# minjiyoon/MMGL

Hardware: AMD Instinct MI355X
Metric: train samples/sec (OPT-1.3B flamingo, 16 neighbors) (higher is better)
Workload: dtype bf16; 1 GPU; opt-1.3b context=all neighbor_mode=embedding peft=flamingo, 11+5 neighbors x 4 tokens, T=512+128, roberta-base + clip-vit-base-patch16 frozen encoders, full train step (fwd+bwd+exchange+AdamW); per_gpu_batch=64, global_batch=64, seq_len=640, neighbor_keys=64, trainable_params=216736520, parallelism=dp1

## Files before the change

include/mmgl_hip.h:

```cpp
#ifndef MMGL_HIP_H
#define MMGL_HIP_H

#include <stddef.h>
#include <stdint.h>

#ifdef __cplusplus
extern "C" {
#endif

enum { MMGL_F32 = 0, MMGL_BF16 = 1 };
enum { MMGL_OK = 0, MMGL_ERR_INVALID = 1, MMGL_ERR_UNSUPPORTED = 2, MMGL_ERR_HIP = 3 };
enum { MMGL_ACT_NONE = 0, MMGL_ACT_RELU = 1 };

const char* mmgl_last_error(void);
int mmgl_version(void);

int mmgl_xattn_fwd(const void* q, const void* k, const void* v, const uint8_t* key_valid,
                   void* out, float* lse, int B, int H, int T, int S, int D, int dtype, void* stream);

size_t mmgl_xattn_bwd_workspace(int B, int H, int T, int S, int D);
int mmgl_xattn_bwd(const void* dout, const void* q, const void* k, const void* v, const float* lse,
                   const uint8_t* key_valid, void* dq, void* dk, void* dv,
                   void* workspace, size_t workspace_bytes,
                   int B, int H, int T, int S, int D, int dtype, void* stream);
// ... 51 lines not shown
size_t mmgl_norm_bwd_workspace(int rows, int cols);
int mmgl_layernorm_bwd(const void* dy, const void* x, const void* gamma, const float* mean, const float* rstd,
                       void* dx, float* dgamma, float* dbeta, void* workspace, size_t workspace_bytes,
                       int rows, int cols, int dtype, void* stream);

int mmgl_rmsnorm_fwd(const void* x, const void* gamma, void* y, float* rstd,
                     int rows, int cols, float eps, int dtype, void* stream);
int mmgl_rmsnorm_bwd(const void* dy, const void* x, const void* gamma, const float* rstd,
                     void* dx, float* dgamma, void* workspace, size_t workspace_bytes,
                     int rows, int cols, int dtype, void* stream);

int mmgl_add_rmsnorm_fwd(const void* x, const void* res, const void* gamma, void* sum_out, void* y, float* rstd,
                         int rows, int cols, float eps, int dtype, void* stream);
int mmgl_add_rmsnorm_bwd(const void* dy, const void* dsum, const void* sum, const void* gamma, const float* rstd,
                         void* dres, float* dgamma, void* workspace, size_t workspace_bytes,
                         int rows, int cols, int dtype, void* stream);

int mmgl_gated_residual_fwd(const void* residual, const void* x, const float* gate, void* y,
                            size_t n, float p_drop, uint64_t seed, int dtype, void* stream);
size_t mmgl_gated_residual_bwd_workspace(size_t n);
int mmgl_gated_residual_bwd(const void* dy, const void* x, const float* gate, void* dx, float* dgate,
                            void* workspace, size_t workspace_bytes,
                            size_t n, float p_drop, uint64_t seed, int dtype, void* stream);

int mmgl_linear_fwd(const void* x, const void* W, const void* bias, void* y,
                    int M, int N, int K, int act, float out_scale, int dtype, void* stream);
size_t mmgl_linear_bwd_workspace(int M, int N, int K, int act, int dtype);
int mmgl_linear_bwd(const void* dy, const void* y, const void* x, const void* W, void* dx, void* dW, void* dbias,
                    void* workspace, size_t workspace_bytes, int M, int N, int K, int act, float out_scale,
                    int accumulate, int mask_dx, int dtype, void* stream);

int mmgl_lora_linear_fwd(const void* x, const void* W, const void* bias, const void* A, const void* Bm,
                         void* y, void* xa, int M, int N, int K, int r, float scale, int dtype, void* stream);
size_t mmgl_lora_linear_bwd_workspace(int M, int N, int K, int r, int dtype);
int mmgl_lora_linear_bwd(const void* dy, const void* x, const void* xa, const void* W, const void* A,
                         const void* Bm, void* dx, void* dA, void* dB, void* dyb, void* workspace,
                         size_t workspace_bytes, int M, int N, int K, int r, float scale, int accumulate,
                         int dtype, void* stream);

int mmgl_neighbor_interleave_fwd(const void* text_emb, const void* vis_emb, const int64_t* text_loc,
                                 const int64_t* img_loc, const int64_t* text_pos, const int64_t* img_pos,
                                 void* out_emb, uint8_t* out_valid, int B, int Nt, int Ni, int n_tok, int d,
                                 int dtype, void* stream);
int mmgl_neighbor_interleave_bwd(const void* d_out_emb, const int64_t* text_loc, const int64_t* img_loc,
                                 void* d_text_emb, void* d_vis_emb, int B, int Nt, int Ni, int n_tok, int d,
                                 int dtype, void* stream);

int mmgl_cross_entropy_fwd(const void* logits, const int64_t* labels, float* row_lse, float* row_loss,
                           float* loss_sum, float* count, int rows, int V, int64_t ignore_index, int dtype,
                           void* stream);
int mmgl_cross_entropy_bwd(const void* logits, const int64_t* labels, const float* row_lse,
                           const float* count, const float* dloss, void* dlogits,
                           int rows, int V, int64_t ignore_index, int dtype, void* stream);

int mmgl_position_ids(const int64_t* attention_mask, int64_t* pos, int B, int T, void* stream);

int mmgl_adamw_step(void* param, float* master, const void* grad, float* exp_avg, float* exp_avg_sq, size_t n,
                    float lr, float beta1, float beta2, float eps, float weight_decay, int step,
                    float grad_scale, int dtype, void* stream);

int mmgl_gemm_nt_fast(int M, int N, int K, int ldx, int ldw, int ldy, int dtype);
size_t mmgl_gemm_nt_workspace(int M, int N, int K, int ldx, int ldw, int ldy, int dtype);
int mmgl_gemm_nt(const void* x, int ldx, const void* W, int ldw, const void* bias, const void* residual, const void* zmask,
                 void* y, int ldy, int M, int N, int K, int act, float out_scale, void* workspace, size_t workspace_bytes,
                 int dtype, void* stream);
int mmgl_relu_bwd(const void* dy, const void* y, void* out, size_t n, int dtype, void* stream);
int mmgl_gemm_nt_rowk(const void* x, int ldx, const void* W, int ldw, void* y, int ldy, int M, int N, int K, int K_short,
                      int m_full, int dtype, void* stream);
int mmgl_gemm_nt_rowk_item(int G, int n_long, int n_short, int q, int wg, int it);
int mmgl_gemm_set_tile_counter(void* counter);
void* mmgl_gemm_get_tile_counter(void);
size_t mmgl_gemm_nt_relu_bits_bytes(int M, int N, int K, int ldx, int ldw, int ldy, int dtype);
int mmgl_gemm_nt_relu_bits(const void* x, int ldx, const void* W, int ldw, const void* bias, void* y, int ldy, void* bits_out,
                           int M, int N, int K, float out_scale, int dtype, void* stream);
int mmgl_gemm_nt_masked(const void* x, int ldx, const void* W, int ldw, const void* bits_in, void* y, int ldy, int M, int N, int K,
                        float out_scale, int dtype, void* stream);

int mmgl_rope_inplace(void* buf, const float* cos_sin, size_t rows, int T, int H, int D, int ld, int nblk, int backward,
                      int dtype, void* stream);
int mmgl_rope(const void* src, void* dst, const float* cos_sin, size_t rows, int T, int H, int D, int ld, int nblk, int nall,
              int backward, int dtype, void* stream);
int mmgl_swiglu_fwd(const void* gate_up, void* y, size_t M, int F, int dtype, void* stream);
int mmgl_swiglu_bwd(const void* dy, const void* gate_up, void* dgate_up, size_t M, int F, int dtype, void* stream);

int mmgl_encattn_fwd(const void* q, const void* k, const void* v, const int32_t* cu_seqlens, void* out, int nseq,
                     int H, int D, int ld_in, int ld_out, int max_len, int q_rows, int dtype, void* stream);
int mmgl_add_layernorm_fwd(const void* x, const void* res, const void* gamma, const void* beta, void* sum_out,
                           void* y, float* mean, float* rstd, int rows, int cols, float eps, float p_drop, uint64_t seed,
                           int dtype, void* stream);
int mmgl_add_layernorm_bwd(const void* dy, const void* dsum, const void* sum, const void* gamma, const float* mean,
                           const float* rstd, void* dres, void* dx, float* dgamma, float* dbeta, void* workspace,
                           size_t workspace_bytes, int rows, int cols, float p_drop, uint64_t seed, int dtype,
                           void* stream);
int mmgl_layernorm_tiles_fwd(const void* x, const void* gamma, const void* beta, void* y, void* yc, const int32_t* rowmap,
                             float* mean, float* rstd, int rows, int cols, int crows, float eps, int dtype, void* stream);
int mmgl_add_layernorm_tiles_fwd(const void* x, const void* res, const void* gamma, const void* beta, void* sum_out, void* y,
                                 void* yc, const int32_t* rowmap, float* mean, float* rstd, int rows, int cols, int crows,
                                 float eps, float p_drop, uint64_t seed, int dtype, void* stream);
int mmgl_add_layernorm_rows_bwd(const void* dy, const int32_t* dy_rows, const void* dsum, const void* sum, const void* gamma,
                                const float* mean, const float* rstd, void* dres, void* dx, float* dgamma, float* dbeta,
                                void* workspace, size_t workspace_bytes, int rows, int cols, float p_drop, uint64_t seed,
                                int dtype, void* stream);
int mmgl_activation_fwd(const void* x, void* y, size_t n, int act, int dtype, void* stream);
int mmgl_scale(const void* x, const float* scale, void* y, size_t n, int dtype, void* stream);

enum { MMGL_COMM_I64 = 2 };
// ... 87 lines not shown
```

mmgl_amd/_lib.py:

```python
import ctypes
import os

import torch

_HERE = os.path.dirname(os.path.abspath(__file__))
LIB_PATH = os.environ.get("MMGL_LIB_PATH") or os.path.join(_HERE, "libmmgl_hip.so")

ABI_VERSION = 110
F32, BF16 = 0, 1
ACT_NONE, ACT_RELU = 0, 1
_ERR_INVALID, _ERR_UNSUPPORTED, _ERR_HIP = 1, 2, 3

c_void_p, c_int, c_float, c_size_t, c_u64, c_i64 = (ctypes.c_void_p, ctypes.c_int, ctypes.c_float, ctypes.c_size_t,
                                                    ctypes.c_uint64, ctypes.c_int64)
P, I, F, Z, U, L = c_void_p, c_int, c_float, c_size_t, c_u64, c_i64

SIGNATURES = {
    "mmgl_last_error": (ctypes.c_char_p, []),
    "mmgl_version": (I, []),
    "mmgl_xattn_fwd": (I, [P, P, P, P, P, P, I, I, I, I, I, I, P]),
    "mmgl_xattn_bwd_workspace": (Z, [I, I, I, I, I]),
    "mmgl_xattn_bwd": (I, [P, P, P, P, P, P, P, P, P, P, Z, I, I, I, I, I, I, P]),
    "mmgl_selfattn_fwd": (I, [P, P, P, P, P, P, I, I, I, I, I, I, P]),
    "mmgl_selfattn_bwd_workspace": (Z, [I, I, I]),
    "mmgl_selfattn_bwd": (I, [P, P, P, P, P, P, P, P, P, P, P, Z, I, I, I, I, I, I, I, P]),
    "mmgl_selfattn_prefix_fwd": (I, [P, P, P, P, P, P, I, I, I, I, I, I, I, I, P]),
    "mmgl_selfattn_prefix_bwd": (I, [P, P, P, P, P, P, P, P, P, P, P, Z, I, I, I, I, I, I, I, I, I, I, P]),
    "mmgl_selfattn_tiles_fwd": (I, [P, P, P, P, P, P, P, I, I, I, I, I, I, I, I, P]),
    "mmgl_selfattn_tiles_bwd": (I, [P, P, P, P, P, P, P, P, P, P, P, P, Z, I, I, I, I, I, I, I, I, I, I, P]),
    "mmgl_selfattn_tiles_rows_bwd": (I, [P, P, P, P, P, P, P, P, P, P, P, P, P, Z, I, I, I, I, I, I, I, I, I, I, I, P]),
    "mmgl_selfattn_gqa_fwd": (I, [P, P, P, P, P, P, I, I, I, I, I, I, I, I, P]),
    "mmgl_selfattn_gqa_bwd_workspace": (Z, [I, I, I, I, I, I]),
    "mmgl_selfattn_gqa_bwd": (I, [P, P, P, P, P, P, P, P, P, P, P, Z, I, I, I, I, I, I, I, I, I, I, P]),
    "mmgl_attn_general_fwd": (I, [P, P, P, P, P, P, P, P, I, I, I, I, I, I, F, U, I, P]),
    "mmgl_attn_general_bwd_workspace": (Z, [I, I, I]),
    "mmgl_attn_general_bwd": (I, [P, P, P, P, P, P, P, P, P, P, P, Z, I, I, I, I, I, I, F, U, I, P]),
    "mmgl_attn_dropout_mask": (I, [P, I, I, I, I, F, U, P]),
    "mmgl_attn_relbias_fwd": (I, [P, P, P, P, P, P, P, P, I, I, I, I, I, I, I, I, I, F, U, I, P]),
    "mmgl_attn_relbias_bwd_workspace": (Z, [I, I, I, I]),
    "mmgl_attn_relbias_bwd": (I, [P, P, P, P, P, P, P, P, P, P, P, P, P, P, Z, I, I, I, I, I, I, I, I, I, F, U, I, P]),
    "mmgl_layernorm_fwd": (I, [P, P, P, P, P, P, I, I, F, I, P]),
    "mmgl_norm_bwd_workspace": (Z, [I, I]),
    "mmgl_layernorm_bwd": (I, [P, P, P, P, P, P, P, P, P, Z, I, I, I, P]),
    "mmgl_rmsnorm_fwd": (I, [P, P, P, P, I, I, F, I, P]),
    "mmgl_rmsnorm_bwd": (I, [P, P, P, P, P, P, P, Z, I, I, I, P]),
    "mmgl_add_rmsnorm_fwd": (I, [P, P, P, P, P, P, I, I, F, I, P]),
    "mmgl_add_rmsnorm_bwd": (I, [P, P, P, P, P, P, P, P, Z, I, I, I, P]),
    "mmgl_gated_residual_fwd": (I, [P, P, P, P, Z, F, U, I, P]),
    "mmgl_gated_residual_bwd_workspace": (Z, [Z]),
    "mmgl_gated_residual_bwd": (I, [P, P, P, P, P, P, Z, Z, F, U, I, P]),
    "mmgl_linear_fwd": (I, [P, P, P, P, I, I, I, I, F, I, P]),
    "mmgl_linear_bwd_workspace": (Z, [I, I, I, I, I]),
    "mmgl_linear_bwd": (I, [P, P, P, P, P, P, P, P, Z, I, I, I, I, F, I, I, I, P]),
    "mmgl_lora_linear_fwd": (I, [P, P, P, P, P, P, P, I, I, I, I, F, I, P]),
    "mmgl_lora_linear_bwd_workspace": (Z, [I, I, I, I, I]),
    "mmgl_lora_linear_bwd": (I, [P, P, P, P, P, P, P, P, P, P, P, Z, I, I, I, I, F, I, I, P]),
    "mmgl_neighbor_interleave_fwd": (I, [P, P, P, P, P, P, P, P, I, I, I, I, I, I, P]),
    "mmgl_neighbor_interleave_bwd": (I, [P, P, P, P, P, I, I, I, I, I, I, P]),
    "mmgl_cross_entropy_fwd": (I, [P, P, P, P, P, P, I, I, L, I, P]),
    "mmgl_cross_entropy_bwd": (I, [P, P, P, P, P, P, I, I, L, I, P]),
    "mmgl_position_ids": (I, [P, P, I, I, P]),
    "mmgl_adamw_step": (I, [P, P, P, P, P, Z, F, F, F, F, F, I, F, I, P]),
    "mmgl_encattn_fwd": (I, [P, P, P, P, P, I, I, I, I, I, I, I, I, P]),
    "mmgl_add_layernorm_fwd": (I, [P, P, P, P, P, P, P, P, I, I, F, F, U, I, P]),
    "mmgl_add_layernorm_bwd": (I, [P, P, P, P, P, P, P, P, P, P, P, Z, I, I, F, U, I, P]),
    "mmgl_layernorm_tiles_fwd": (I, [P, P, P, P, P, P, P, P, I, I, I, F, I, P]),
    "mmgl_add_layernorm_tiles_fwd": (I, [P, P, P, P, P, P, P, P, P, P, I, I, I, F, F, U, I, P]),
    "mmgl_activation_fwd": (I, [P, P, Z, I, I, P]),
    "mmgl_scale": (I, [P, P, P, Z, I, P]),
    "mmgl_gemm_nt_fast": (I, [I, I, I, I, I, I, I]),
    "mmgl_gemm_nt_workspace": (Z, [I, I, I, I, I, I, I]),
    "mmgl_gemm_nt_relu_bits_bytes": (Z, [I, I, I, I, I, I, I]),
    "mmgl_gemm_nt_relu_bits": (I, [P, I, P, I, P, P, I, P, I, I, I, F, I, P]),
    "mmgl_gemm_nt_masked": (I, [P, I, P, I, P, P, I, I, I, I, F, I, P]),
    "mmgl_gemm_nt": (I, [P, I, P, I, P, P, P, P, I, I, I, I, I, F, P, Z, I, P]),
    "mmgl_gemm_nt_rowk": (I, [P, I, P, I, P, I, I, I, I, I, I, I, P]),
    "mmgl_gemm_nt_rowk_item": (I, [I, I, I, I, I, I]),
    "mmgl_add_layernorm_rows_bwd": (I, [P, P, P, P, P, P, P, P, P, P, P, P, Z, I, I, F, U, I, P]),
    "mmgl_relu_bwd": (I, [P, P, P, Z, I, P]),
    "mmgl_gemm_set_tile_counter": (I, [P]),
    "mmgl_gemm_get_tile_counter": (P, []),
    "mmgl_rope_inplace": (I, [P, P, Z, I, I, I, I, I, I, I, P]),
    "mmgl_rope": (I, [P, P, P, Z, I, I, I, I, I, I, I, I, P]),
    "mmgl_swiglu_fwd": (I, [P, P, Z, I, I, P]),
    "mmgl_swiglu_bwd": (I, [P, P, P, Z, I, I, P]),
    "mmgl_comm_unique_id": (I, [P]),
    "mmgl_comm_init": (I, [I, I, P, ctypes.POINTER(ctypes.c_void_p)]),
    "mmgl_allreduce_sum": (I, [P, P, Z, I, P]),
    "mmgl_allgather": (I, [P, P, P, Z, I, P]),
    "mmgl_broadcast": (I, [P, P, Z, I, I, P]),
    "mmgl_comm_destroy": (I, [P]),
    "mmgl_gemm_skinny": (I, [P, I, P, I, P, P, P, I, I, I, I, I, F, I, P]),
    "mmgl_attn_decode_fwd": (I, [P, I, P, P, I, Z, P, I, P, I, I, I, I, I, P]),
    "mmgl_gemm_skinny_lora": (I, [P, I, P, I, P, P, P, I, P, I, P, I, I, F, P, I, I, I, I, F, I, P]),
    "mmgl_attn_decode_gqa_fwd": (I, [P, I, P, P, I, Z, P, I, P, I, I, I, I, I, I, P]),
    "mmgl_rope_kv_append": (I, [P, I, P, P, Z, I, I, I, I, I, P]),
    "mmgl_attn_decode_beam_fwd": (I, [P, I, P, P, I, Z, P, I, P, P, I, Z, P, I, P, I, I, I, I, I, I, I, P]),
    "mmgl_beam_topk_workspace": (Z, [I, I, I]),
    "mmgl_beam_topk": (I, [P, Z, P, P, P, P, Z, I, I, I, I, I, P]),
    "mmgl_beam_advance": (I, [P, P, P, P, P, P, P, I, P, P, P, P, P, P, P, P, P, I, I, I, I, I, I, I, F, P]),
    "mmgl_sample_tokens": (I, [P, Z, P, P, L, P, P, I, I, I, F, I, F, I, L, I, P]),
    "mmgl_logits_process": (I, [P, Z, P, Z, P, Z, I, I, P, I, I, I, F, I, I, P]),
    "mmgl_guidance_logits": (I, [P, Z, I, I, F, I, P]),
    "mmgl_attn_decode_block_fwd": (I, [P, I, P, P, I, P, P, I, Z, I, P, I, P, P, I, I, I, I, I, P]),
    "mmgl_lookup_accept": (I, [P, Z, I, P, P, P, P, Z, P, Z, P, P, P, P, I, I, I, I, I, I, L, L, I, I, I, P]),
    "mmgl_rope_kv_append_block": (I, [P, I, P, I, P, I, Z, I, P, I, I, I, I, I, I, P]),
    "mmgl_attn_decode_gqa_block_fwd": (I, [P, I, P, P, I, Z, I, P, I, P, P, I, I, I, I, I, I, P]),
    "mmgl_contrastive_chunk": (I, []),
    "mmgl_contrastive_workspace": (Z, [I, I, I]),
    "mmgl_contrastive_select": (I, [P, Z, P, Z, Z, P, Z, I, P, P, Z, F, I, I, P, Z, P, Z, P, L, L, P, P, P, P, P, P, Z, I, I, I, I, I, P]),
    "mmgl_kv_quantize": (I, [P, P, I, Z, P, I, Z, P, I, Z, I, I, I, I, I, P]),
    "mmgl_attn_decode_q8_fwd": (I, [P, I, P, P, I, P, P, I, Z, P, P, I, Z, I, P, I, P, I, I, I, I, I, P]),
    "mmgl_attn_decode_gqa_q8_fwd": (I, [P, I, P, P, I, P, P, I, Z, P, P, I, Z, I, P, I, P, I, I, I, I, I, I, P]),
# ... 42 lines not shown


def ptr(t):
    return None if t is None else ctypes.c_void_p(t.data_ptr())


def ptr_off(t, nbytes):
    return ctypes.c_void_p(t.data_ptr() + int(nbytes))


_raw_stream = getattr(torch._C, "_cuda_getCurrentRawStream", None)
_raw_device = getattr(torch._C, "_cuda_getDevice", None)


def stream_ptr():
    if _raw_stream is not None and _raw_device is not None:
        return ctypes.c_void_p(_raw_stream(_raw_device()))
    return ctypes.c_void_p(torch.cuda.current_stream().cuda_stream)


def require_cuda(*ts):
    for t in ts:
        if t is not None and not t.is_cuda:
            raise RuntimeError("mmgl_amd ops run on the GPU only (tensor is on %s); there is no CPU path" % t.device)


class KernelTimer:
    enabled = False
    only = None
    records = []
    by_tag = bool(os.environ.get("MMGL_KERNEL_TAGS"))

    @classmethod
    def reset(cls):
        cls.records = []

    @classmethod
    def summary(cls):
        torch.cuda.synchronize()
        out = {}
        for name, s, e, work in cls.records:
            if cls.by_tag and "tag" in work:
                name = f"{name}[{work['tag']}]"
            d = out.setdefault(name, dict(calls=0, ms_total=0.0, bytes=0.0, flops=0.0))
            d["calls"] += 1
            d["ms_total"] += s.elapsed_time(e)
            d["bytes"] += work.get("bytes", 0.0)
            d["flops"] += work.get("flops", 0.0)
        for d in out.values():
            d["ms_avg"] = d["ms_total"] / d["calls"]
        return out


def call(name: str, work, *args):
    fn = getattr(lib(), name)
    if KernelTimer.enabled and (KernelTimer.only is None or name in KernelTimer.only):
        s = torch.cuda.Event(enable_timing=True)
        e = torch.cuda.Event(enable_timing=True)
        s.record()
        rc = fn(*args)
        e.record()
        KernelTimer.records.append((name, s, e, work() if callable(work) else (work or {})))
    else:
        rc = fn(*args)
    check(rc, name)
```

mmgl_amd/csrc/elementwise.hip:

```cpp
#include "common.h"

namespace {

template <typename T> struct Vec {
    static constexpr int N = 16 / sizeof(T);
    typedef T type __attribute__((ext_vector_type(16 / sizeof(T))));
};

__device__ __forceinline__ float block_sum(float v, float* red) {
    v = wave_sum(v);
    __syncthreads();
    if ((threadIdx.x & 63) == 0) red[threadIdx.x >> 6] = v;
    __syncthreads();
    return red[0] + red[1] + red[2] + red[3];
}
__device__ __forceinline__ float block_max(float v, float* red) {
    v = wave_max(v);
    __syncthreads();
    if ((threadIdx.x & 63) == 0) red[threadIdx.x >> 6] = v;
    __syncthreads();
    return fmaxf(fmaxf(red[0], red[1]), fmaxf(red[2], red[3]));
}

inline int stream_blocks(size_t nvec) {
// ... 211 lines not shown

__global__ __launch_bounds__(256) void ce_finish_kernel(const float* __restrict__ row_loss, const int64_t* __restrict__ labels,
                                                        int rows, int V_, int64_t ignore, float* __restrict__ loss_sum,
                                                        float* __restrict__ count) {
    __shared__ float red[4];
    float a = 0.f, c = 0.f;
    for (int i = threadIdx.x; i < rows; i += 256) {
        const int64_t lab = labels[i];
        if (!(lab == ignore || lab < 0 || lab >= V_)) { a += row_loss[i]; c += 1.f; }
    }
    const float sa = block_sum(a, red);
    const float sc = block_sum(c, red);
    if (threadIdx.x == 0) { *loss_sum = sa; *count = sc; }
}

template <typename T>
__global__ __launch_bounds__(256) void ce_bwd_kernel(const T* __restrict__ logits, const int64_t* __restrict__ labels,
                                                     const float* __restrict__ row_lse, const float* __restrict__ count,
                                                     const float* __restrict__ dloss, T* __restrict__ dlogits, int V_,
                                                     int64_t ignore) {
    typedef typename Vec<T>::type V;
    constexpr int VN = Vec<T>::N;
    const int row = blockIdx.x;
    const T* x = logits + (size_t)row * V_;
    T* dx = dlogits + (size_t)row * V_;
    const int64_t lab = labels[row];
    const bool ign = (lab == ignore || lab < 0 || lab >= V_);
    const float scale = ign ? 0.f : (*dloss) / fmaxf(*count, 1.f);
    const float lse = row_lse[row];
    const int nvec = (((size_t)V_ * sizeof(T)) % 16 == 0) ? V_ / VN : 0;
    auto grad = [&](int i, const V& v) __attribute__((always_inline)) {
        V o;
#pragma unroll
        for (int j = 0; j < VN; ++j) {
            float g = __expf((float)v[j] - lse);
            if (i * VN + j == lab) g -= 1.f;
            o[j] = (T)(g * scale);
        }
        ((V*)dx)[i] = o;
    };
    int i = threadIdx.x;
    for (; i + 768 < nvec; i += 1024) {
        const V v0 = ((const V*)x)[i], v1 = ((const V*)x)[i + 256], v2 = ((const V*)x)[i + 512], v3 = ((const V*)x)[i + 768];
        grad(i, v0);
        grad(i + 256, v1);
        grad(i + 512, v2);
        grad(i + 768, v3);
    }
    for (; i < nvec; i += 256) grad(i, ((const V*)x)[i]);
    for (int i = nvec * VN + threadIdx.x; i < V_; i += 256) {
        float g = __expf((float)x[i] - lse);
        if (i == lab) g -= 1.f;
        dx[i] = (T)(g * scale);
    }
}

__global__ __launch_bounds__(64) void position_ids_kernel(const int64_t* __restrict__ mask, int64_t* __restrict__ pos, int T_) {
    const int b = blockIdx.x, lane = threadIdx.x;
    int64_t carry = 0;
    for (int t0 = 0; t0 < T_; t0 += 64) {
        const int t = t0 + lane;
        const int64_t m = t < T_ ? mask[(size_t)b * T_ + t] : 0;
        int64_t v = m;
#pragma unroll
        for (int o = 1; o < 64; o <<= 1) {
            const int64_t u = __shfl_up(v, o);
            if (lane >= o) v += u;
        }
        if (t < T_) pos[(size_t)b * T_ + t] = (carry + v) * m - 1 + 2;
        carry += __shfl(v, 63);
    }
}

template <typename T>
__global__ __launch_bounds__(256) void adamw_kernel(T* __restrict__ param, float* __restrict__ master,
                                                    const T* __restrict__ grad, float* __restrict__ m,
                                                    float* __restrict__ v, size_t n, float lr, float b1, float b2,
                                                    float eps, float wd, float bc1, float bc2s, float gscale) {
    for (size_t i = (size_t)blockIdx.x * 256 + threadIdx.x; i < n; i += (size_t)gridDim.x * 256) {
        const float g = (float)grad[i] * gscale;
        float p = master ? master[i] : (float)param[i];
        p *= 1.f - lr * wd;
        const float mi = b1 * m[i] + (1.f - b1) * g;
        const float vi = b2 * v[i] + (1.f - b2) * g * g;
        m[i] = mi;
        v[i] = vi;
        p -= (lr / bc1) * mi / (sqrtf(vi) / bc2s + eps);
        if (master) master[i] = p;
        param[i] = (T)p;
    }
}

}

#define BY_DTYPE(CALL_BF16, CALL_F32, who)                        \
    do {                                                          \
        if (dtype == MMGL_BF16) { CALL_BF16; }                    \
        else if (dtype == MMGL_F32) { CALL_F32; }                 \
        else MMGL_FAIL(MMGL_ERR_INVALID, "%s: bad dtype %d", who, dtype); \
    } while (0)

extern "C" int mmgl_gated_residual_fwd(const void* residual, const void* x, const float* gate, void* y, size_t n,
                                       float p_drop, uint64_t seed, int dtype, void* stream) {
    MMGL_CHECK_ARG(residual && x && y, "mmgl_gated_residual_fwd: null pointer");
    MMGL_CHECK_ARG(p_drop >= 0.f && p_drop < 1.f, "mmgl_gated_residual_fwd: dropout p=%g outside [0,1)", p_drop);
    if (n == 0) return MMGL_OK;
// ... 55 lines not shown
}

extern "C" int mmgl_neighbor_interleave_bwd(const void* d_out_emb, const int64_t* text_loc, const int64_t* img_loc,
                                            void* d_text_emb, void* d_vis_emb, int B, int Nt, int Ni, int n_tok, int d,
                                            int dtype, void* stream) {
    MMGL_CHECK_ARG(B > 0 && Nt >= 0 && Ni >= 0 && Nt + Ni > 0 && n_tok > 0 && d > 0, "mmgl_neighbor_interleave_bwd: bad sizes");
    MMGL_CHECK_ARG(d_out_emb && (Nt == 0 || (d_text_emb && text_loc)) && (Ni == 0 || (d_vis_emb && img_loc)),
                   "mmgl_neighbor_interleave_bwd: null pointer");
    MMGL_CHECK_ARG(n_tok <= 256, "mmgl_neighbor_interleave_bwd: n_tok > 256");
    MMGL_CHECK_ARG(dtype == MMGL_BF16 || dtype == MMGL_F32, "mmgl_neighbor_interleave_bwd: bad dtype %d", dtype);
    const size_t esz = dtype == MMGL_BF16 ? 2 : 4;
    if (((size_t)n_tok * d * esz) % 16) MMGL_FAIL(MMGL_ERR_UNSUPPORTED, "mmgl_neighbor_interleave_bwd: n_tok*d must cover whole 16-byte chunks");
    hipStream_t st = (hipStream_t)stream;
    const int N = Nt + Ni;
    BY_DTYPE(hipLaunchKernelGGL(interleave_bwd_kernel<bf16>, dim3(B * N), dim3(256), 0, st, (const bf16*)d_out_emb, text_loc,
                                img_loc, (bf16*)d_text_emb, (bf16*)d_vis_emb, Nt, Ni, n_tok, d),
             hipLaunchKernelGGL(interleave_bwd_kernel<float>, dim3(B * N), dim3(256), 0, st, (const float*)d_out_emb, text_loc,
                                img_loc, (float*)d_text_emb, (float*)d_vis_emb, Nt, Ni, n_tok, d),
             "mmgl_neighbor_interleave_bwd");
    MMGL_CHECK_LAUNCH("mmgl_neighbor_interleave_bwd");
    return MMGL_OK;
}

extern "C" int mmgl_cross_entropy_fwd(const void* logits, const int64_t* labels, float* row_lse, float* row_loss,
                                      float* loss_sum, float* count, int rows, int V, int64_t ignore_index, int dtype,
                                      void* stream) {
    MMGL_CHECK_ARG(logits && labels && row_lse && row_loss && loss_sum && count, "mmgl_cross_entropy_fwd: null pointer");
    MMGL_CHECK_ARG(rows > 0 && V > 0, "mmgl_cross_entropy_fwd: bad sizes");
    hipStream_t st = (hipStream_t)stream;
    BY_DTYPE(hipLaunchKernelGGL(ce_fwd_kernel<bf16>, dim3(rows), dim3(256), 0, st, (const bf16*)logits, labels, row_lse,
                                row_loss, V, ignore_index),
             hipLaunchKernelGGL(ce_fwd_kernel<float>, dim3(rows), dim3(256), 0, st, (const float*)logits, labels, row_lse,
                                row_loss, V, ignore_index),
             "mmgl_cross_entropy_fwd");
    hipLaunchKernelGGL(ce_finish_kernel, dim3(1), dim3(256), 0, st, row_loss, labels, rows, V, ignore_index, loss_sum, count);
    MMGL_CHECK_LAUNCH("mmgl_cross_entropy_fwd");
    return MMGL_OK;
}

extern "C" int mmgl_cross_entropy_bwd(const void* logits, const int64_t* labels, const float* row_lse, const float* count,
                                      const float* dloss, void* dlogits, int rows, int V, int64_t ignore_index, int dtype,
                                      void* stream) {
    MMGL_CHECK_ARG(logits && labels && row_lse && count && dloss && dlogits, "mmgl_cross_entropy_bwd: null pointer");
    hipStream_t st = (hipStream_t)stream;
    BY_DTYPE(hipLaunchKernelGGL(ce_bwd_kernel<bf16>, dim3(rows), dim3(256), 0, st, (const bf16*)logits, labels, row_lse, count,
                                dloss, (bf16*)dlogits, V, ignore_index),
             hipLaunchKernelGGL(ce_bwd_kernel<float>, dim3(rows), dim3(256), 0, st, (const float*)logits, labels, row_lse,
                                count, dloss, (float*)dlogits, V, ignore_index),
             "mmgl_cross_entropy_bwd");
    MMGL_CHECK_LAUNCH("mmgl_cross_entropy_bwd");
    return MMGL_OK;
}

extern "C" int mmgl_position_ids(const int64_t* attention_mask, int64_t* pos, int B, int T, void* stream) {
    MMGL_CHECK_ARG(attention_mask && pos && B > 0 && T > 0, "mmgl_position_ids: bad arguments");
    hipLaunchKernelGGL(position_ids_kernel, dim3(B), dim3(64), 0, (hipStream_t)stream, attention_mask, pos, T);
    MMGL_CHECK_LAUNCH("mmgl_position_ids");
    return MMGL_OK;
}

extern "C" int mmgl_adamw_step(void* param, float* master, const void* grad, float* exp_avg, float* exp_avg_sq, size_t n,
                               float lr, float beta1, float beta2, float eps, float weight_decay, int step,
                               float grad_scale, int dtype, void* stream) {
    MMGL_CHECK_ARG(param && grad && exp_avg && exp_avg_sq && step >= 1, "mmgl_adamw_step: bad arguments");
    if (n == 0) return MMGL_OK;
    const float bc1 = (float)(1.0 - pow((double)beta1, (double)step));
    const float bc2s = (float)sqrt(1.0 - pow((double)beta2, (double)step));
    hipStream_t st = (hipStream_t)stream;
    const int blocks = stream_blocks(n);
    BY_DTYPE(hipLaunchKernelGGL(adamw_kernel<bf16>, dim3(blocks), dim3(256), 0, st, (bf16*)param, master, (const bf16*)grad,
                                exp_avg, exp_avg_sq, n, lr, beta1, beta2, eps, weight_decay, bc1, bc2s, grad_scale),
             hipLaunchKernelGGL(adamw_kernel<float>, dim3(blocks), dim3(256), 0, st, (float*)param, master, (const float*)grad,
                                exp_avg, exp_avg_sq, n, lr, beta1, beta2, eps, weight_decay, bc1, bc2s, grad_scale),
             "mmgl_adamw_step");
    MMGL_CHECK_LAUNCH("mmgl_adamw_step");
    return MMGL_OK;
}

template <typename T> static int act_launch(const void* x, void* y, size_t n, int act, hipStream_t st) {
    const int blocks = stream_blocks(n / (16 / sizeof(T)));
    switch (act) {
        case 1: hipLaunchKernelGGL((act_kernel<T, 1>), dim3(blocks), dim3(256), 0, st, (const T*)x, (T*)y, n); break;
        case 2: hipLaunchKernelGGL((act_kernel<T, 2>), dim3(blocks), dim3(256), 0, st, (const T*)x, (T*)y, n); break;
        case 3: hipLaunchKernelGGL((act_kernel<T, 3>), dim3(blocks), dim3(256), 0, st, (const T*)x, (T*)y, n); break;
        default: hipLaunchKernelGGL((act_kernel<T, 4>), dim3(blocks), dim3(256), 0, st, (const T*)x, (T*)y, n); break;
    }
    MMGL_CHECK_LAUNCH("mmgl_activation_fwd");
    return MMGL_OK;
}

extern "C" int mmgl_activation_fwd(const void* x, void* y, size_t n, int act, int dtype, void* stream) {
    MMGL_CHECK_ARG(x && y, "mmgl_activation_fwd: null pointer");
    MMGL_CHECK_ARG(act >= 1 && act <= 4, "mmgl_activation_fwd: act %d not in {1 relu, 2 gelu, 3 quick_gelu, 4 gelu_tanh}", act);
    if (n == 0) return MMGL_OK;
    hipStream_t st = (hipStream_t)stream;
    if (dtype == MMGL_BF16) return act_launch<bf16>(x, y, n, act, st);
    if (dtype == MMGL_F32) return act_launch<float>(x, y, n, act, st);
    MMGL_FAIL(MMGL_ERR_INVALID, "mmgl_activation_fwd: bad dtype %d", dtype);
}

extern "C" int mmgl_scale(const void* x, const float* scale, void* y, size_t n, int dtype, void* stream) {
    MMGL_CHECK_ARG(x && y && scale, "mmgl_scale: null pointer");
    if (n == 0) return MMGL_OK;
    hipStream_t st = (hipStream_t)stream;
    if (dtype == MMGL_BF16) hipLaunchKernelGGL(scale_kernel<bf16>, dim3(stream_blocks(n / 8)), dim3(256), 0, st, (const bf16*)x, scale, (bf16*)y, n);
    else if (dtype == MMGL_F32) hipLaunchKernelGGL(scale_kernel<float>, dim3(stream_blocks(n / 4)), dim3(256), 0, st, (const float*)x, scale, (float*)y, n);
// ... 5 lines not shown
```

mmgl_amd/model/modelling_cross_attention.py:

```python
import math
import os
from typing import List, Optional, Tuple, Union

import torch
import torch.nn as nn
import torch.nn.functional as F
from transformers import (AutoConfig, AutoModelForCausalLM, CLIPTextModel, CLIPVisionModel, PretrainedConfig,
                          RobertaModel)
from transformers.activations import ACT2FN
from transformers.modeling_outputs import BaseModelOutputWithPast, CausalLMOutputWithPast

from .. import ops
from .decode_cache import BeamState, DecodeCache, LookupState, StepCodes
from .encoders import ClipTextEncoder, PackedTextEncoder, PackedVisionEncoder
from .generation import beam_loop, check_prompt, contrastive_loop, decode_loop, lookup_loop, make_select
from .sampling import (check_contrastive, check_guidance, check_kv_cache, check_lookup, check_processors, check_sampling,
                       check_weight_dtype)

CROSS_MODES = ("cross_attention", "embedding")


def uses_cross_attention(neighbor_mode: str, peft_type: str = "flamingo") -> bool:
    return neighbor_mode == "cross_attention" or (neighbor_mode == "embedding" and peft_type == "flamingo")

# ... 743 lines not shown
        return h

    def _verify_step(self, cache):
        lookup = cache.lookup
        if lookup is None or cache.beam is not None or cache.next_pos is None:
            raise ValueError("a verify step needs a prefilled DecodeCache with a LookupState (cache.lookup) and no BeamState")
        ops.require_cuda(cache.mask)
        with torch.no_grad():
            return self._decode_rows(self.embed_tokens(lookup.block.view(-1)), lookup.positions.view(-1), cache)


class MPTModel(MPTPreTrainedModel):
    def __init__(self, config: MPTConfig):
        super().__init__(config)
        self.decoder = MPTDecoder(config)

    def get_input_embeddings(self):
        return self.decoder.embed_tokens

    def set_input_embeddings(self, value):
        self.decoder.embed_tokens = value

    def get_decoder(self):
        return self.decoder

    def forward(self, *args, **kwargs):
        return self.decoder(*args, **kwargs)


def reset_peft_parameters(model):
    for n, p in model.named_parameters():
        if "lora_A" in n:
            nn.init.kaiming_uniform_(p, a=math.sqrt(5))
        if "lora_B" in n:
            nn.init.zeros_(p)


def mark_only_peft_as_trainable(model):
    for p in model.parameters():
        p.requires_grad = False
    for m in model.modules():
        if isinstance(m, MPTDecoderLayer) and m.cross_attention:
            for p in m.parameters():
                p.requires_grad = True


def lm_head_loss_and_logits(module, lm_head, hidden, next_labels, return_logits=None, logits_slice=None):
    frozen = type(lm_head) is nn.Linear and not lm_head.weight.requires_grad and lm_head.bias is None
    lanes = 16 // hidden.element_size()
    aligned = lm_head.weight.shape[0] % lanes == 0 and lm_head.weight.shape[1] % lanes == 0
    opted_out = return_logits is False or (return_logits is None and logits_slice is not None)
    fuse = next_labels is not None and frozen and hidden.is_cuda and opted_out and aligned
    if fuse:
        loss = ops.lm_head_cross_entropy(hidden, lm_head.weight, next_labels)
        logits = None
        if logits_slice is not None:
            with torch.no_grad():
                logits = _lin(lm_head, hidden.detach()[:, logits_slice].contiguous())
        return loss, logits
    logits = _lin(lm_head, hidden)
    loss = None
    if next_labels is not None:
        loss = ops.cross_entropy(logits.view(-1, logits.shape[-1]), next_labels.view(-1))
    if logits_slice is not None:
        logits = logits[:, logits_slice]
    return loss, logits


class MPTForCausalLM(MPTPreTrainedModel):
    _tied_weights_keys = ["lm_head.weight"]

    def __init__(self, config):
        super().__init__(config)
        self.model = MPTModel(config)
        self.lm_head = nn.Linear(config.word_embed_proj_dim, config.vocab_size, bias=False)
        self.lm_head.apply(self._init_weights)
        self.lm_head.weight = self.model.decoder.embed_tokens.weight
        if config.peft_type != "none":
            reset_peft_parameters(self.model)
            mark_only_peft_as_trainable(self.model)

    def get_input_embeddings(self):
        return self.model.decoder.embed_tokens

    def set_input_embeddings(self, value):
        self.model.decoder.embed_tokens = value

    def get_output_embeddings(self):
        return self.lm_head

    def set_output_embeddings(self, new_embeddings):
        self.lm_head = new_embeddings

    def set_decoder(self, decoder):
        self.model.decoder = decoder

    def get_decoder(self):
        return self.model.decoder

    def forward(self, input_ids=None, attention_mask=None, head_mask=None, past_key_values=None, inputs_embeds=None,
                labels=None, neighbor_embeds=None, neighbor_attention_mask=None, use_cache=None, output_attentions=None,
                output_hidden_states=None, return_dict=None, first_key_valid=False, return_logits=None, logits_slice=None,
                cache_capacity=None, key_tiles=None, kv_cache_dtype=None):
        return_dict = True if return_dict is None else return_dict
        outputs = self.model.decoder(input_ids=input_ids, attention_mask=attention_mask, head_mask=head_mask,
                                     past_key_values=past_key_values, inputs_embeds=inputs_embeds,
                                     neighbor_embeds=neighbor_embeds, neighbor_attention_mask=neighbor_attention_mask,
                                     use_cache=use_cache, output_attentions=output_attentions,
                                     output_hidden_states=output_hidden_states, return_dict=True, first_key_valid=first_key_valid,
# ... 457 lines not shown
```

mmgl_amd/ops.py:

```python
import math
import os
import weakref

import torch
import torch.nn.functional as F

from . import _lib
from ._lib import dtype_code, lib, ptr, ptr_off, require_cuda, stream_ptr


def _dropout(p_drop, training, seed):
    p = float(p_drop) if training else 0.0
    if p > 0.0 and seed is None:
        seed = int(torch.randint(0, 2 ** 62, (1,)).item())
    return p, int(seed or 0)


def _check_mask(key_valid, shape):
    if key_valid.shape != shape:
        raise ValueError(f"Attention mask should be of size {tuple(shape)}, but is {tuple(key_valid.shape)}")


def _key_valid(key_valid):
    if key_valid.dtype != torch.uint8:
# ... 998 lines not shown
        ctx.mark_non_differentiable(valid)
        return out, valid

    @staticmethod
    def backward(ctx, dout, _dvalid):
        tl, il = ctx.saved_tensors
        B, Nt, Ni, n_tok, d = ctx.dims
        dout = dout.contiguous()
        dtext = torch.empty(B, Nt, n_tok, d, dtype=dout.dtype, device=dout.device)
        dvis = torch.empty(B, Ni, n_tok, d, dtype=dout.dtype, device=dout.device) if Ni else None
        _lib.call("mmgl_neighbor_interleave_bwd", None, ptr(dout), ptr(tl), ptr(il), ptr(dtext), ptr(dvis), B, Nt, Ni, n_tok, d,
                                                 dtype_code(dout), stream_ptr())
        return dtext, dvis, None, None, None, None


def neighbor_interleave(text_emb, vis_emb, text_loc, img_loc, text_pos, img_pos):
    if vis_emb is not None and vis_emb.shape[2:] != text_emb.shape[2:]:
        raise ValueError("n_text_tokens must equal n_visual_tokens for the interleaved layout (reference :1083-1098)")
    return _Interleave.apply(text_emb, vis_emb, text_loc, img_loc, text_pos, img_pos)


class _CrossEntropy(torch.autograd.Function):
    @staticmethod
    def forward(ctx, logits, labels, ignore_index):
        require_cuda(logits, labels)
        rows, V = logits.shape
        logits = logits.contiguous()
        labels = labels.contiguous()
        dev = logits.device
        row_lse = torch.empty(rows, dtype=torch.float32, device=dev)
        row_loss = torch.empty(rows, dtype=torch.float32, device=dev)
        sums = torch.empty(2, dtype=torch.float32, device=dev)
        _lib.call("mmgl_cross_entropy_fwd", dict(bytes=1.0 * rows * V * logits.element_size()), ptr(logits), ptr(labels), ptr(row_lse), ptr(row_loss), ptr(sums[0:1]), ptr(sums[1:2]),
                                           rows, V, ignore_index, dtype_code(logits), stream_ptr())
        ctx.save_for_backward(logits, labels, row_lse, sums)
        ctx.ignore = ignore_index
        return sums[0] / sums[1]

    @staticmethod
    def backward(ctx, dloss):
        logits, labels, row_lse, sums = ctx.saved_tensors
        rows, V = logits.shape
        dl = dloss.detach().to(torch.float32).reshape(1).contiguous()
        dlogits = torch.empty_like(logits)
        _lib.call("mmgl_cross_entropy_bwd", dict(bytes=2.0 * rows * V * logits.element_size()), ptr(logits), ptr(labels), ptr(row_lse), ptr(sums[1:2]), ptr(dl), ptr(dlogits), rows, V,
                                           ctx.ignore, dtype_code(logits), stream_ptr())
        return dlogits, None, None


def cross_entropy(logits, labels, ignore_index=-100):
    return _CrossEntropy.apply(logits, labels, int(ignore_index))


class _LMHeadCrossEntropy(torch.autograd.Function):

    @staticmethod
    def forward(ctx, hidden, weight, labels, ignore_index, chunk_rows):
        require_cuda(hidden, weight, labels)
        V, d = weight.shape
        h2 = hidden.reshape(-1, d)
        if not h2.is_contiguous():
            h2 = h2.contiguous()
        M = h2.shape[0]
        lab = labels.reshape(-1).contiguous()
        dev = h2.device
        w = weight if weight.dtype == h2.dtype else weight.to(h2.dtype)
        count = (lab != ignore_index).sum().to(torch.float32).reshape(1)
        one = torch.ones(1, dtype=torch.float32, device=dev)
        loss_sum = torch.zeros(1, dtype=torch.float32, device=dev)
        dh = torch.empty_like(h2)
        chunk = min(M, int(chunk_rows))
        scratch = torch.empty(chunk, V, dtype=h2.dtype, device=dev)
        row_lse = torch.empty(chunk, dtype=torch.float32, device=dev)
        row_loss = torch.empty(chunk, dtype=torch.float32, device=dev)
        part = torch.empty(2, dtype=torch.float32, device=dev)
        code = dtype_code(h2)
        es = h2.element_size()
        for r0 in range(0, M, chunk):
            r1 = min(M, r0 + chunk)
            n = r1 - r0
            lg = scratch[:n]
            gemm_nt(h2[r0:r1], w.contiguous(), out=lg)
            _lib.call("mmgl_cross_entropy_fwd", dict(bytes=1.0 * n * V * es), ptr(lg), ptr(lab[r0:r1]), ptr(row_lse), ptr(row_loss), ptr(part[0:1]),
                      ptr(part[1:2]), n, V, ignore_index, code, stream_ptr())
            loss_sum += part[0:1]
            _lib.call("mmgl_cross_entropy_bwd", dict(bytes=2.0 * n * V * es), ptr(lg), ptr(lab[r0:r1]), ptr(row_lse), ptr(count), ptr(one), ptr(lg), n, V,
                      ignore_index, code, stream_ptr())
            frozen_dgrad(lg, weight, out=dh[r0:r1])
        ctx.save_for_backward(dh)
        ctx.shape = hidden.shape
        return (loss_sum / count.clamp_min(1.0)).reshape(())

    @staticmethod
    def backward(ctx, dloss):
        (dh,) = ctx.saved_tensors
        s = dloss.detach().to(torch.float32).reshape(1).contiguous()
        out = torch.empty_like(dh)
        _lib.call("mmgl_scale", dict(bytes=2.0 * dh.numel() * dh.element_size()), ptr(dh), ptr(s), ptr(out), dh.numel(), dtype_code(dh),
                  stream_ptr())
        return out.view(ctx.shape), None, None, None, None


def lm_head_cross_entropy(hidden, weight, labels, ignore_index=-100, chunk_rows=8192):
    if weight.requires_grad:
        raise ValueError("lm_head_cross_entropy: the head must be frozen (use lm_head + cross_entropy for a trainable head)")
    if hidden.shape[:-1] != labels.shape or hidden.shape[-1] != weight.shape[1]:
        raise ValueError(f"lm_head_cross_entropy: shapes hidden{tuple(hidden.shape)} weight{tuple(weight.shape)} labels{tuple(labels.shape)}")
    return _LMHeadCrossEntropy.apply(hidden, weight, labels, int(ignore_index), int(chunk_rows))


def position_ids(attention_mask):
    require_cuda(attention_mask)
    m = attention_mask.to(torch.int64).contiguous()
    out = torch.empty_like(m)
    _lib.call("mmgl_position_ids", None, ptr(m), ptr(out), m.shape[0], m.shape[1], stream_ptr())
    return out


def adamw_step_(param, master, grad, exp_avg, exp_avg_sq, lr, beta1, beta2, eps, weight_decay, step, grad_scale=1.0):
    require_cuda(param, grad)
    _lib.call("mmgl_adamw_step", None, ptr(param), ptr(master), ptr(grad), ptr(exp_avg), ptr(exp_avg_sq), param.numel(), lr, beta1, beta2,
                                eps, weight_decay, step, grad_scale, dtype_code(param), stream_ptr())


_WT_CACHE = {}
ACT_CODES = {"none": 0, "relu": 1, "gelu": 2, "quick_gelu": 3, "gelu_new": 4, "gelu_pytorch_tanh": 4, "gelu_fast": 4}


def _padded_t(weight, pad_to=1):
    with torch.no_grad():
        wt = weight.detach().t()
        n = wt.shape[1]
        npad = (n + pad_to - 1) // pad_to * pad_to
        if npad == n:
            return wt.contiguous()
        full = wt.new_zeros(wt.shape[0], npad)
        full[:, :n] = wt
        return full


def _transposed(weight, pad_to=1):
    key = (id(weight), pad_to)
    tag = (weight.data_ptr(), weight._version, weight.dtype, tuple(weight.shape))
    hit = _WT_CACHE.get(key)
    if hit is None or hit[0]() is not weight or hit[1] != tag:
        if len(_WT_CACHE) > 4096:
            for k in [k for k, h in _WT_CACHE.items() if h[0]() is None]:
                del _WT_CACHE[k]
        hit = (weakref.ref(weight), tag, _padded_t(weight, pad_to))
        _WT_CACHE[key] = hit
    return hit[2]


_tile_counters = {}


def gemm_dynamic_schedule(enable=True, device=None):
    device = torch.device("cuda", torch.cuda.current_device()) if device is None else torch.device(device)
    with torch.cuda.device(device):
        if not enable:
            lib().mmgl_gemm_set_tile_counter(None)
# ... 1049 lines not shown
```

Before: 281.3 samples/s.

## Fuse cross-entropy forward and backward into one register-resident kernel with slice capture

Replaces the separate cross-entropy forward and backward launches on each lm-head logits chunk with a single kernel. It holds a row's logits in registers, computes an online max and sum, then writes the gradient in place, so logits are read from memory once instead of twice. The same kernel can also copy a requested slice of logits, which avoids recomputing the sliced logits with an extra lm-head GEMM. The cost is heavy register use (a cap of 32 vectors per thread), bf16-only support with a fallback path, and an extra autograd output.

```diff
diff --git a/include/mmgl_hip.h b/include/mmgl_hip.h
--- a/include/mmgl_hip.h
+++ b/include/mmgl_hip.h
@@ -127,6 +127,11 @@
 int mmgl_cross_entropy_bwd(const void* logits, const int64_t* labels, const float* row_lse,
                            const float* count, const float* dloss, void* dlogits,
                            int rows, int V, int64_t ignore_index, int dtype, void* stream);
+
+int mmgl_cross_entropy_fused(const void* logits, const int64_t* labels, float* row_lse, float* row_loss,
+                             float* loss_sum, float* count, const float* total, const float* dloss, void* dlogits,
+                             void* slice_out, int rows, int V, int64_t ignore_index, int64_t row0, int T, int t0, int t1,
+                             int dtype, void* stream);
 
 int mmgl_position_ids(const int64_t* attention_mask, int64_t* pos, int B, int T, void* stream);
 
diff --git a/mmgl_amd/_lib.py b/mmgl_amd/_lib.py
--- a/mmgl_amd/_lib.py
+++ b/mmgl_amd/_lib.py
@@ -59,6 +59,7 @@
     "mmgl_neighbor_interleave_bwd": (I, [P, P, P, P, P, I, I, I, I, I, I, P]),
     "mmgl_cross_entropy_fwd": (I, [P, P, P, P, P, P, I, I, L, I, P]),
     "mmgl_cross_entropy_bwd": (I, [P, P, P, P, P, P, I, I, L, I, P]),
+    "mmgl_cross_entropy_fused": (I, [P, P, P, P, P, P, P, P, P, P, I, I, L, L, I, I, I, I, P]),
     "mmgl_position_ids": (I, [P, P, I, I, P]),
     "mmgl_adamw_step": (I, [P, P, P, P, P, Z, F, F, F, F, F, I, F, I, P]),
     "mmgl_encattn_fwd": (I, [P, P, P, P, P, I, I, I, I, I, I, I, I, P]),
@@ -207,7 +208,7 @@
         return out
 
 
-def call(name: str, work, *args):
+def _invoke(name, work, args):
     fn = getattr(lib(), name)
     if KernelTimer.enabled and (KernelTimer.only is None or name in KernelTimer.only):
         s = torch.cuda.Event(enable_timing=True)
@@ -215,7 +216,19 @@
         s.record()
         rc = fn(*args)
         e.record()
-        KernelTimer.records.append((name, s, e, work() if callable(work) else (work or {})))
-    else:
-        rc = fn(*args)
+        if rc == 0:
+            KernelTimer.records.append((name, s, e, work() if callable(work) else (work or {})))
+        return rc
+    return fn(*args)
+
+
+def call(name: str, work, *args):
+    check(_invoke(name, work, args), name)
+
+
+def call_or_refuse(name: str, work, *args):
+    rc = _invoke(name, work, args)
+    if rc == _ERR_UNSUPPORTED:
+        return False
     check(rc, name)
+    return True
diff --git a/mmgl_amd/csrc/elementwise.hip b/mmgl_amd/csrc/elementwise.hip
--- a/mmgl_amd/csrc/elementwise.hip
+++ b/mmgl_amd/csrc/elementwise.hip
@@ -287,6 +287,88 @@
         float g = __expf((float)x[i] - lse);
         if (i == lab) g -= 1.f;
         dx[i] = (T)(g * scale);
+    }
+}
+
+template <typename T, int CAP>
+__global__ __launch_bounds__(256) void ce_fused_kernel(const T* logits, const int64_t* __restrict__ labels,
+                                                       float* __restrict__ row_lse, float* __restrict__ row_loss,
+                                                       const float* __restrict__ count, const float* __restrict__ dloss, T* dlogits,
+                                                       T* slice_out, int V_, int64_t ignore, int64_t row0, int T_, int t0, int t1) {
+    typedef typename Vec<T>::type V;
+    constexpr int VN = Vec<T>::N;
+    __shared__ float red[4];
+    const int row = blockIdx.x;
+    const V* x = (const V*)(logits + (size_t)row * V_);
+    const int nvec = V_ / VN;
+    const int tid = threadIdx.x, nk = (nvec - tid + 255) >> 8;
+    V r[CAP];
+#pragma unroll
+    for (int k = 0; k < CAP; ++k)
+        if (k < nk) r[k] = (x + 256 * k)[tid];
+    float m = -INFINITY, s = 0.f;
+    auto fold = [&](const V& v, bool fused) __attribute__((always_inline)) {
+        float lm = (float)v[0];
+#pragma unroll
+        for (int j = 1; j < VN; ++j) lm = fmaxf(lm, (float)v[j]);
+        const float nm = fmaxf(m, lm);
+        const float sh = nm == -INFINITY ? 0.f : nm;
+        float acc = 0.f;
+#pragma unroll
+        for (int j = 0; j < VN; ++j) acc += __expf((float)v[j] - sh);
+        const float e = __expf(m - sh);
+        float plain;
+        {
+#pragma clang fp contract(off)
+            const float p = s * e;
+            plain = p + acc;
+        }
+        s = fused ? __builtin_fmaf(s, e, acc) : plain;
+        m = nm;
+    };
+#pragma unroll
+    for (int k = 0; k < CAP; ++k)
+        if (k < nk) fold(r[k], (k & 1) || (k | 3) >= nk);
+#pragma unroll
+    for (int k = 0; k < CAP; ++k) asm volatile("" : "+v"(r[k]));
+    const float gm = block_max(m, red);
+    const float gs = block_sum(m == -INFINITY ? 0.f : s * __expf(m - gm), red);
+    const float lse = gm + logf(gs);
+    const int64_t lab = labels[row];
+    const bool ign = (lab == ignore || lab < 0 || lab >= V_);
+    if (tid == 0) {
+        row_lse[row] = lse;
+        if (ign) row_loss[row] = 0.f;
+    }
+    if (slice_out) {
+        const int64_t mrow = row0 + row, b = mrow / T_;
+        const int t = (int)(mrow - b * T_);
+        if (t >= t0 && t < t1) {
+            V* so = (V*)(slice_out + ((size_t)b * (t1 - t0) + (t - t0)) * V_);
+#pragma unroll
+            for (int k = 0; k < CAP; ++k)
+                if (k < nk) (so + 256 * k)[tid] = r[k];
+        }
+    }
+    const float scale = ign ? 0.f : (*dloss) / fmaxf(*count, 1.f);
+    V* dx = (V*)(dlogits + (size_t)row * V_);
+#pragma unroll
+    for (int k = 0; k < CAP; ++k) {
+        if (k < nk) {
+            const int i = tid + 256 * k;
+            const V v = r[k];
+            V o;
+#pragma unroll
+            for (int j = 0; j < VN; ++j) {
+                float g = __expf((float)v[j] - lse);
+                if (i * VN + j == lab) {
+                    g -= 1.f;
+                    if (!ign) row_loss[row] = lse - (float)v[j];
+                }
+                o[j] = (T)(g * scale);
+            }
+            (dx + 256 * k)[tid] = o;
+        }
     }
 }
 
@@ -448,6 +530,29 @@
     return MMGL_OK;
 }
 
+extern "C" int mmgl_cross_entropy_fused(const void* logits, const int64_t* labels, float* row_lse, float* row_loss, float* loss_sum,
+                                        float* count, const float* total, const float* dloss, void* dlogits, void* slice_out,
+                                        int rows, int V, int64_t ignore_index, int64_t row0, int T, int t0, int t1, int dtype,
+                                        void* stream) {
+    constexpr int CAP = 32;
+    MMGL_CHECK_ARG(logits && labels && row_lse && row_loss && loss_sum && count && total && dloss && dlogits,
+                   "mmgl_cross_entropy_fused: null pointer");
+    MMGL_CHECK_ARG(rows > 0 && V > 0, "mmgl_cross_entropy_fused: bad sizes");
+    MMGL_CHECK_ARG(dtype == MMGL_BF16 || dtype == MMGL_F32, "mmgl_cross_entropy_fused: bad dtype %d", dtype);
+    MMGL_CHECK_ARG(!slice_out || (row0 >= 0 && T > 0 && 0 <= t0 && t0 <= t1 && t1 <= T),
+                   "mmgl_cross_entropy_fused: bad slice (row0 %lld, T %d, t0 %d, t1 %d)", (long long)row0, T, t0, t1);
+    if (dtype != MMGL_BF16) MMGL_FAIL(MMGL_ERR_UNSUPPORTED, "mmgl_cross_entropy_fused: bf16 only");
+    if (V % 8 || ((uintptr_t)logits | (uintptr_t)dlogits | (uintptr_t)slice_out) % 16)
+        MMGL_FAIL(MMGL_ERR_UNSUPPORTED, "mmgl_cross_entropy_fused: rows are not 16-byte aligned (V = %d)", V);
+    if (V / 8 > 256 * CAP) MMGL_FAIL(MMGL_ERR_UNSUPPORTED, "mmgl_cross_entropy_fused: V = %d > %d", V, 8 * 256 * CAP);
+    hipStream_t st = (hipStream_t)stream;
+    hipLaunchKernelGGL((ce_fused_kernel<bf16, CAP>), dim3(rows), dim3(256), 0, st, (const bf16*)logits, labels, row_lse, row_loss, total,
+                       dloss, (bf16*)dlogits, (bf16*)slice_out, V, ignore_index, row0, T, t0, t1);
+    hipLaunchKernelGGL(ce_finish_kernel, dim3(1), dim3(256), 0, st, row_loss, labels, rows, V, ignore_index, loss_sum, count);
+    MMGL_CHECK_LAUNCH("mmgl_cross_entropy_fused");
+    return MMGL_OK;
+}
+
 extern "C" int mmgl_position_ids(const int64_t* attention_mask, int64_t* pos, int B, int T, void* stream) {
     MMGL_CHECK_ARG(attention_mask && pos && B > 0 && T > 0, "mmgl_position_ids: bad arguments");
     hipLaunchKernelGGL(position_ids_kernel, dim3(B), dim3(64), 0, (hipStream_t)stream, attention_mask, pos, T);
diff --git a/mmgl_amd/model/modelling_cross_attention.py b/mmgl_amd/model/modelling_cross_attention.py
--- a/mmgl_amd/model/modelling_cross_attention.py
+++ b/mmgl_amd/model/modelling_cross_attention.py
@@ -819,9 +819,16 @@
     opted_out = return_logits is False or (return_logits is None and logits_slice is not None)
     fuse = next_labels is not None and frozen and hidden.is_cuda and opted_out and aligned
     if fuse:
-        loss = ops.lm_head_cross_entropy(hidden, lm_head.weight, next_labels)
-        logits = None
-        if logits_slice is not None:
+        rows = None
+        if isinstance(logits_slice, slice) and hidden.dim() == 3:
+            t0, t1, step = logits_slice.indices(hidden.shape[1])
+            if step == 1:
+                rows = (hidden.shape[1], t0, max(t0, t1))
+        if rows is None:
+            loss, logits = ops.lm_head_cross_entropy(hidden, lm_head.weight, next_labels), None
+        else:
+            loss, logits = ops.lm_head_cross_entropy(hidden, lm_head.weight, next_labels, slice_rows=rows)
+        if logits is None and logits_slice is not None:
             with torch.no_grad():
                 logits = _lin(lm_head, hidden.detach()[:, logits_slice].contiguous())
         return loss, logits
diff --git a/mmgl_amd/ops.py b/mmgl_amd/ops.py
--- a/mmgl_amd/ops.py
+++ b/mmgl_amd/ops.py
@@ -1074,10 +1074,15 @@
     return _CrossEntropy.apply(logits, labels, int(ignore_index))
 
 
+def lm_head_slice_row(m, T, t0, t1):
+    b, t = divmod(m, T)
+    return b * (t1 - t0) + (t - t0) if t0 <= t < t1 else None
+
+
 class _LMHeadCrossEntropy(torch.autograd.Function):
 
     @staticmethod
-    def forward(ctx, hidden, weight, labels, ignore_index, chunk_rows):
+    def forward(ctx, hidden, weight, labels, ignore_index, chunk_rows, slice_rows):
         require_cuda(hidden, weight, labels)
         V, d = weight.shape
         h2 = hidden.reshape(-1, d)
@@ -1098,37 +1103,61 @@
         part = torch.empty(2, dtype=torch.float32, device=dev)
         code = dtype_code(h2)
         es = h2.element_size()
+        T, t0, t1 = slice_rows if slice_rows is not None else (1, 0, 0)
+        sl = torch.empty(M // T, t1 - t0, V, dtype=h2.dtype, device=dev) if slice_rows is not None else None
+        fused = None
         for r0 in range(0, M, chunk):
             r1 = min(M, r0 + chunk)
             n = r1 - r0
             lg = scratch[:n]
             gemm_nt(h2[r0:r1], w.contiguous(), out=lg)
-            _lib.call("mmgl_cross_entropy_fwd", dict(bytes=1.0 * n * V * es), ptr(lg), ptr(lab[r0:r1]), ptr(row_lse), ptr(row_loss), ptr(part[0:1]),
-                      ptr(part[1:2]), n, V, ignore_index, code, stream_ptr())
-            loss_sum += part[0:1]
-            _lib.call("mmgl_cross_entropy_bwd", dict(bytes=2.0 * n * V * es), ptr(lg), ptr(lab[r0:r1]), ptr(row_lse), ptr(count), ptr(one), ptr(lg), n, V,
-                      ignore_index, code, stream_ptr())
+            if fused is not False:
+                work = lambda: dict(bytes=(2.0 * n + (_slice_rows_in(r0, r1, T, t0, t1) if sl is not None else 0)) * V * es)
+                fused = _lib.call_or_refuse("mmgl_cross_entropy_fused", work, ptr(lg), ptr(lab[r0:r1]), ptr(row_lse), ptr(row_loss),
+                                            ptr(part[0:1]), ptr(part[1:2]), ptr(count), ptr(one), ptr(lg), ptr(sl), n, V, ignore_index,
+                                            r0, T, t0, t1, code, stream_ptr())
+                if fused:
+                    loss_sum += part[0:1]
+            if not fused:
+                _lib.call("mmgl_cross_entropy_fwd", dict(bytes=1.0 * n * V * es), ptr(lg), ptr(lab[r0:r1]), ptr(row_lse), ptr(row_loss), ptr(part[0:1]),
+                          ptr(part[1:2]), n, V, ignore_index, code, stream_ptr())
+                loss_sum += part[0:1]
+                _lib.call("mmgl_cross_entropy_bwd", dict(bytes=2.0 * n * V * es), ptr(lg), ptr(lab[r0:r1]), ptr(row_lse), ptr(count), ptr(one), ptr(lg), n, V,
+                          ignore_index, code, stream_ptr())
             frozen_dgrad(lg, weight, out=dh[r0:r1])
         ctx.save_for_backward(dh)
         ctx.shape = hidden.shape
-        return (loss_sum / count.clamp_min(1.0)).reshape(())
-
-    @staticmethod
-    def backward(ctx, dloss):
+        loss = (loss_sum / count.clamp_min(1.0)).reshape(())
+        if not fused or sl is None:
+            return loss, None
+        ctx.mark_non_differentiable(sl)
+        return loss, sl
+
+    @staticmethod
+    def backward(ctx, dloss, _dslice=None):
         (dh,) = ctx.saved_tensors
         s = dloss.detach().to(torch.float32).reshape(1).contiguous()
         out = torch.empty_like(dh)
         _lib.call("mmgl_scale", dict(bytes=2.0 * dh.numel() * dh.element_size()), ptr(dh), ptr(s), ptr(out), dh.numel(), dtype_code(dh),
                   stream_ptr())
-        return out.view(ctx.shape), None, None, None, None
-
-
-def lm_head_cross_entropy(hidden, weight, labels, ignore_index=-100, chunk_rows=8192):
+        return out.view(ctx.shape), None, None, None, None, None
+
+
+def _slice_rows_in(r0, r1, T, t0, t1):
+    return sum(max(0, min(r1, b * T + t1) - max(r0, b * T + t0)) for b in range(r0 // T, (r1 - 1) // T + 1))
+
+
+def lm_head_cross_entropy(hidden, weight, labels, ignore_index=-100, chunk_rows=8192, slice_rows=None):
     if weight.requires_grad:
         raise ValueError("lm_head_cross_entropy: the head must be frozen (use lm_head + cross_entropy for a trainable head)")
     if hidden.shape[:-1] != labels.shape or hidden.shape[-1] != weight.shape[1]:
         raise ValueError(f"lm_head_cross_entropy: shapes hidden{tuple(hidden.shape)} weight{tuple(weight.shape)} labels{tuple(labels.shape)}")
-    return _LMHeadCrossEntropy.apply(hidden, weight, labels, int(ignore_index), int(chunk_rows))
+    if slice_rows is not None:
+        T, t0, t1 = (int(v) for v in slice_rows)
+        if not (T > 0 and 0 <= t0 <= t1 <= T and labels.numel() % T == 0):
+            raise ValueError(f"lm_head_cross_entropy: slice_rows {tuple(slice_rows)} does not fit {labels.numel()} rows")
+        return _LMHeadCrossEntropy.apply(hidden, weight, labels, int(ignore_index), int(chunk_rows), (T, t0, t1))
+    return _LMHeadCrossEntropy.apply(hidden, weight, labels, int(ignore_index), int(chunk_rows), None)[0]
 
 
 def position_ids(attention_mask):
```

New measurement: 279.6 samples/s (median of 2 runs). About the same (-0.6%).
